# vincenthz/eccoxide

Hardware: AMD Instinct MI355X
Metric: variable-base scalarmuls/sec (batch) per GPU + achieved HBM GB/s vs roofline (higher is better)
Workload: dtype u32

## Files before the change

__graft_entry__.py:

```python
import os
import subprocess
import sys

ROOT = os.path.dirname(os.path.abspath(__file__))
if ROOT not in sys.path:
    sys.path.insert(0, ROOT)


def build() -> None:
    jobs = str(min(6, os.cpu_count() or 1))
    subprocess.check_call(["make", "-C", os.path.join(ROOT, "eccoxide_amd", "csrc"), "-j", jobs, "ARCH=gfx950"])
    subprocess.check_call(["make", "-C", os.path.join(ROOT, "oracle")])
    subprocess.check_call(["make", "-C", os.path.join(ROOT, "tests", "cpp")])
    subprocess.check_call(["make", "-C", os.path.join(ROOT, "tests", "hip")])
    subprocess.check_call(["make", "-C", os.path.join(ROOT, "tests", "hip_p256k1")])
    subprocess.check_call(["make", "-C", os.path.join(ROOT, "tests", "hip_ed25519")])
    subprocess.check_call(["make", "-C", os.path.join(ROOT, "tests", "hip_merged")])
    subprocess.check_call(["make", "-C", os.path.join(ROOT, "tests", "hip_signed")])
    subprocess.check_call(["make", "-C", os.path.join(ROOT, "tests", "hip_lo32")])
    subprocess.check_call(["make", "-C", os.path.join(ROOT, "tests", "hip_ecdsa")])
    subprocess.check_call(["make", "-C", os.path.join(ROOT, "tests", "hip_ed25519_sign")])
    subprocess.check_call(["make", "-C", os.path.join(ROOT, "tests", "hip_ecdsa_sign")])
    subprocess.check_call(["make", "-C", os.path.join(ROOT, "tests", "hip_h2c")])
    subprocess.check_call(["make", "-C", os.path.join(ROOT, "tests", "hip_g2")])
    subprocess.check_call(["make", "-C", os.path.join(ROOT, "tests", "hip_h2c_g2")])
    import eccoxide_amd
    from eccoxide_amd import _lib

    lib = _lib.load()
    assert lib.eccx_field_bytes(eccoxide_amd.P256R1) == 32


def smoke() -> None:
    import eccoxide_amd as E
    from eccoxide_amd import workload as W
    from tests import oracle_lib

    ora = oracle_lib.load()
    with E.Engine(0) as eng:
        for curve, n in (("p256r1", 300), ("ed25519", 300)):
            ks = W.random_scalars(curve, n, seed=1).tobytes()
            want_b = ora.base(curve, ks, threads=4)
            got_b = eng.scalarmul_base(curve, ks)
            assert got_b[0] == want_b[0] and got_b[1] == want_b[1], f"{curve}: fixed-base mismatch vs oracle"
            pts = want_b[0]
            ks2 = W.random_scalars(curve, n, seed=2).tobytes()
            want_v = ora.var(curve, ks2, pts, threads=4)
            got_d = eng.scalarmul_var(curve, ks2, pts)
            assert got_d[0] == want_v[0] and got_d[1] == want_v[1], f"{curve}: variable-base mismatch vs oracle"
            got_v = eng.scalarmul_var(curve, ks2, pts, want_proj=True)
            assert got_v[0] == want_v[0] and got_v[1] == want_v[1], f"{curve}: mirror variable-base mismatch vs oracle"
            assert got_v[2] == want_v[2], f"{curve}: un-normalised coordinates differ from the reference algorithm"
            for kw in ({"ct_scan": True}, {"ct_gather": True}):
                got_c = eng.scalarmul_base(curve, ks, **kw)
                assert got_c[0] == want_b[0] and got_c[1] == want_b[1], f"{curve} {kw}: secret-scalar fixed base mismatch vs oracle"
            got_c = eng.scalarmul_var(curve, ks2, pts, ct_scan=True)
            assert got_c[0] == want_v[0] and got_c[1] == want_v[1], f"{curve}: secret-scalar variable base mismatch vs oracle"
            from oracle import ecc_ref as R

            inf = None if curve == "ed25519" else got_d[1]
            enc = eng.point_compress(curve, got_d[0], inf)
            assert enc == R.point_compress_bytes(curve, got_d[0], inf), f"{curve}: point encoding differs from the oracle"
            back = eng.point_decompress(curve, enc)
            assert back[0] == got_d[0] and back[1] == (bytes(n) if inf is None else inf), f"{curve}: decompress(compress(P)) != P"
        curve, n = "bls12_381_g1", 200
        pts = ora.base(curve, W.random_scalars(curve, n, seed=3).tobytes(), threads=4)[0]
        ks = W.random_scalars(curve, n, seed=4).tobytes()
        want = ora.var(curve, ks, pts, threads=4)
        for opts in ({}, {"assume_subgroup": True}, {"ct_scan": True}, {"ct_scan": True, "assume_subgroup": True}):
            got = eng.scalarmul_var(curve, ks, pts, **opts)
            assert got[0] == want[0] and got[1] == want[1], f"{curve} {opts}: variable-base mismatch vs oracle"
# ... 58 lines not shown
```

eccoxide_amd/csrc/kernels_coz.hpp:

```cpp
#pragma once
#include <type_traits>
#include "inv_gcd.hpp"
#include "kernels_ct.hpp"

namespace eccx {

struct NoGlv {
  static constexpr int K_BITS = 0;
};
struct PrimeOrderBases : NoGlv {};

template <class G>
ECCX_DEV void glv_split(uint32_t (&k1)[5], uint32_t (&k2)[5], const uint8_t* __restrict__ kb) {
  uint32_t k[8];
#pragma unroll
  for (int i = 0; i < 8; ++i) {
    const uint8_t* b = kb + 28 - 4 * i;
    k[i] = ((uint32_t)b[0] << 24) | ((uint32_t)b[1] << 16) | ((uint32_t)b[2] << 8) | (uint32_t)b[3];
  }
  uint32_t prod[13];
#pragma unroll
  for (int i = 0; i < 13; ++i) prod[i] = 0;
#pragma unroll
  for (int i = 0; i < 8; ++i) {
// ... 156 lines not shown
    }
  }
  s1 = h1[4] >> 31;
  s2 = h2[4] >> 31;
  uint32_t c_1 = s1, c_2 = s2;
#pragma unroll
  for (int i = 0; i < 5; ++i) {
    const uint64_t a = (uint64_t)(h1[i] ^ (0u - s1)) + c_1;
    k1[i] = (uint32_t)a;
    c_1 = (uint32_t)(a >> 32);
    const uint64_t b = (uint64_t)(h2[i] ^ (0u - s2)) + c_2;
    k2[i] = (uint32_t)b;
    c_2 = (uint32_t)(b >> 32);
  }
}


template <class CU>
constexpr int urowc_words() { return ((3 * CU::N + 3) / 4) * 4; }

template <class CU>
ECCX_DEV void u2_load(U<CU, 1, 3>& x, U<CU, 1, 3>& y, const uint32_t* __restrict__ row) {
  constexpr int N = CU::N;
  constexpr int W = ((2 * N + 3) / 4) * 4;
  uint32_t w[W];
  const uint4* src = reinterpret_cast<const uint4*>(row);
#pragma unroll
  for (int i = 0; i < W / 4; ++i) {
    const uint4 q = src[i];
    w[4 * i] = q.x; w[4 * i + 1] = q.y; w[4 * i + 2] = q.z; w[4 * i + 3] = q.w;
  }
#pragma unroll
  for (int i = 0; i < N; ++i) { x.v[i] = w[i]; y.v[i] = w[N + i]; }
}

template <class CU>
constexpr int urow2_words() { return ((2 * CU::N + 3) / 4) * 4; }
#ifndef ECCX_CT_VAR_PK
#define ECCX_CT_VAR_PK 0
#endif
template <class CU, bool TAGGED = false>
ECCX_DEV void u2_store(uint32_t* __restrict__ row, const U<CU, 1, 3>& x, const U<CU, 1, 3>& y) {
  constexpr int N = CU::N;
  constexpr int W = urow2_words<CU>();
  constexpr uint32_t T = TAGGED ? CT_F32_TAG : 0u;
  uint32_t w[W];
#pragma unroll
  for (int i = 0; i < W; ++i) w[i] = (i < N ? x.v[i] : (i < 2 * N ? y.v[i - N] : 0u)) | T;
  uint4* dst = reinterpret_cast<uint4*>(row);
#pragma unroll
  for (int i = 0; i < W / 4; ++i) dst[i] = make_uint4(w[4 * i], w[4 * i + 1], w[4 * i + 2], w[4 * i + 3]);
}

template <class CU>
ECCX_DEV void ujac_madd_signed(UJac<CU>& r, bool& h_zero, bool& r_zero, const UJac<CU>& p,
                          const U<CU, 1, 3>& x2, const U<CU, 1, 3>& y2, bool neg) {
  auto z1z1 = u_sqr(p.z);
  auto u2 = u_mul(x2, z1z1);
  auto t = u_mul(p.z, z1z1);
  U<CU, 2, 4> sy;
  u_select(sy, neg, u_neg(y2), u_as<2, 4>(y2));
  auto s2 = u_mul(u_reduce(sy), t);
  auto h = u_reduce(u_sub(u2, p.x));
  auto rr = u_reduce(u_sub(s2, p.y));
  h_zero = u_is_zero_mod_p(h);
  r_zero = u_is_zero_mod_p(rr);
  auto hh = u_sqr(h);
  auto hhh = u_mul(h, hh);
  auto v = u_mul(p.x, hh);
  auto r2 = u_sqr(rr);
  auto x3 = u_reduce(u_sub(u_sub(u_sub(r2, hhh), v), v));
  r.x = x3;
  if constexpr (CU::KIND == UK_MONT) {
    r.y = u_fit<1, 3>(u_mul_add(rr, u_sub(v, x3), u_neg(p.y), hhh));
  } else if constexpr (UB<CU>::SPARSE) {
    r.y = u_mul_sub(rr, u_sub(v, x3), p.y, hhh);
  } else if constexpr (UBS<CU>::DENSE) {
    r.y = u_mul_sub(rr, u_sdiff(v, x3), p.y, hhh);
  } else {
    auto y3a = u_mul(rr, u_sub(v, x3));
    auto y1h = u_mul(p.y, hhh);
    r.y = u_reduce(u_sub(y3a, y1h));
  }
  r.z = u_fit<UJac<CU>::ZK, UJac<CU>::ZV>(u_mul(p.z, h));
}

template <class CU>
ECCX_DEV void uzaddu(U<CU, 1, 3>& x1, U<CU, 1, 3>& y1, U<CU, 1, 3>& x2, U<CU, 1, 3>& y2, U<CU, 1, 3>& d_out, bool& d_zero) {
  const auto d = u_reduce(u_sub(x1, x2));
  d_zero = u_is_zero_mod_p(d);
  const auto c = u_sqr(d);
  const U<CU, 1, 3> w1 = u_fit<1, 3>(u_mul(x1, c));
  const auto w2 = u_mul(x2, c);
  const auto e = u_reduce(u_sub(y1, y2));
  const auto dd = u_sqr(e);
  const U<CU, 1, 3> a1 = u_fit<1, 3>(u_mul(y1, u_sub(w1, w2)));
  const auto x3 = u_reduce(u_sub(u_sub(dd, w1), w2));
  const auto y3m = u_mul(e, u_sub(w1, x3));
  x2 = x3;
  y2 = u_reduce(u_sub(y3m, a1));
  x1 = w1;
  y1 = a1;
  d_out = d;
}

template <class CU>
ECCX_DEV void ujac_madd_ct(UJac<CU>& r, bool& h_zero, bool& r_zero, const UJac<CU>& p, const U<CU, 1, 3>& x2,
                           const U<CU, 1, 3>& y2) {
  auto z1z1 = u_sqr(p.z);
  auto u2 = u_mul(x2, z1z1);
  auto t = u_mul(p.z, z1z1);
  auto s2 = u_mul(y2, t);
  auto h = u_reduce(u_sub(u2, p.x));
  auto rr = u_reduce(u_sub(s2, p.y));
  h_zero = u_is_zero_mod_p_ct(h);
  r_zero = u_is_zero_mod_p_ct(rr);
  auto hh = u_sqr(h);
  auto hhh = u_mul(h, hh);
  auto v = u_mul(p.x, hh);
  auto r2 = u_sqr(rr);
  auto x3 = u_reduce(u_sub(u_sub(u_sub(r2, hhh), v), v));
  r.x = x3;
  if constexpr (CU::KIND == UK_MONT) {
    r.y = u_fit<1, 3>(u_mul_add(rr, u_sub(v, x3), u_neg(p.y), hhh));
  } else if constexpr (UB<CU>::SPARSE) {
    r.y = u_mul_sub(rr, u_sub(v, x3), p.y, hhh);
  } else {
    auto y3a = u_mul(rr, u_sub(v, x3));
    auto y1h = u_mul(p.y, hhh);
    r.y = u_reduce(u_sub(y3a, y1h));
  }
  r.z = u_fit<UJac<CU>::ZK, UJac<CU>::ZV>(u_mul(p.z, h));
}

template <class CU>
ECCX_DEV void ujac_dbl_affine(U<CU, 1, 3>& x3, U<CU, 1, 3>& y3, U<CU, 1, 3>& z3, U<CU, 1, 3>& sv, U<CU, 1, 3>& y8v,
                              const U<CU, 1, 3>& px, const U<CU, 1, 3>& py) {
// ... 28 lines not shown
  constexpr int NWIN = (8 * CS::SB + 1 + WB - 1) / WB;
  return (CS::PRIME_ORDER || ASSUME_PRIME) ? (8 * CS::SB - CS::NBITS + 1) / WB + 1 : NWIN;
}
#ifndef ECCX_CT_VAR_BITS
#define ECCX_CT_VAR_BITS 4
#endif

#ifndef ECCX_COZ_OCC_U14
#define ECCX_COZ_OCC_U14 3
#endif
#ifndef ECCX_COZ_OCC_BLS
#define ECCX_COZ_OCC_BLS 2
#endif
#ifndef ECCX_COZ_OCC_U9
#define ECCX_COZ_OCC_U9 4
#endif
#ifndef ECCX_COZ_NESTED_LADDER
#define ECCX_COZ_NESTED_LADDER 1
#endif
template <class CU, bool GLV>
constexpr int coz_occupancy() {
  return CU::N <= 9 ? ECCX_COZ_OCC_U9
                    : (CU::N <= 14 ? (GLV ? ECCX_OCC_U14 : (CU::KIND == UK_MONT ? ECCX_COZ_OCC_BLS : ECCX_COZ_OCC_U14)) : ECCX_OCC_U18);
}


template <class CU, class G, bool GLV, bool FUSED = false, int WB = 5, bool CT = false>
__global__ void __launch_bounds__(WG, (coz_occupancy<CU, GLV>())) k_scalarmul_coz_unsat(size_t n, const uint8_t* __restrict__ scalars,
                                                                                 const uint8_t* __restrict__ points,
                                                                                 uint32_t* __restrict__ rows_out,
                                                                                 uint8_t* __restrict__ flags,
                                                                                 uint32_t* __restrict__ scratch, uint32_t opts,
                                                                                 const uint8_t* __restrict__ base_scalars = nullptr,
                                                                                 const uint32_t* __restrict__ utable = nullptr) {
  static_assert(!(GLV && FUSED), "the verify shape takes any curve point");
  static_assert(!(CT && FUSED), "the verify shape has no secret-scalar form");
  constexpr bool ASSUME_PRIME = std::is_same<G, PrimeOrderBases>::value;
  constexpr bool LATTICE = GlvLattice<G>::value;
  static_assert(!(LATTICE && CT), "the secret-scalar endomorphism ladder is written for the unsigned split");
  static_assert(!ASSUME_PRIME || CT, "PrimeOrderBases only narrows the secret-scalar form's collision windows");
  static_assert(WB >= 3 && WB <= 5, "table rows 1 .. 2^(WB-1) must fit the slab");
  constexpr int TBL = 1 << (WB - 1);
  using CS = typename CU::Sat;
  constexpr bool ISO = CS::A0 == 1;
  constexpr int L = CS::L;
  constexpr int N = CU::N;
  constexpr int FB = CS::FB;
  constexpr int SB = CS::SB;
  static_assert(!GLV || SB == 32, "the split is written for 256-bit scalars");
  constexpr int NWIN = GLV ? (G::K_BITS + 1 + WB - 1) / WB : (8 * SB + 1 + WB - 1) / WB;
  constexpr int S = (!GLV && !CT) ? (8 * SB + 1) % WB : 0;
  constexpr int NWIN_MAIN = S != 0 ? (8 * SB + 1) / WB : NWIN;
  constexpr bool SHARED_INV = !ISO && !CT;
  static_assert(WG == 256, "the shared inversion multiplies the values of four waves");
  constexpr int WR = urowc_words<CU>();
  static_assert(!ISO || WR >= 16 + N, "row 0 holds the split scalar and zeta");
  using T = U<CU, 1, 3>;
  uint32_t* slab = scratch + ((size_t)blockIdx.x * FAST_TABLE_ROWS * WG + threadIdx.x) * (size_t)WR;
  auto row = [&](uint32_t e) { return slab + (size_t)e * WG * WR; };
  constexpr int WC = urow2_words<CU>();
  static_assert(!CT || (size_t)TBL * WC <= (size_t)(FAST_TABLE_ROWS - 1 - TBL) * WR, "the compact table must fit the free rows");
  uint32_t* cslab = scratch + ((size_t)blockIdx.x * FAST_TABLE_ROWS + (TBL + 1)) * WG * (size_t)WR + (size_t)threadIdx.x * WC;
  auto crow = [&](uint32_t e) { return cslab + (size_t)(e - 1) * WG * WC; };
  uint32_t iter = 0u;
  for (size_t base = (size_t)blockIdx.x * WG; base < n; base += (size_t)gridDim.x * WG, ++iter) {
    const size_t gid = base + threadIdx.x;
    const bool active = gid < n;
    const size_t idx = active ? gid : n - 1;
    const uint8_t* __restrict__ k = scalars + idx * (size_t)SB;
    if constexpr (GLV) {
      uint32_t k1[5], k2[5], s1 = 0, s2 = 0;
      if constexpr (LATTICE) glv_split_lattice<G>(k1, k2, s1, s2, k);
      else glv_split<G>(k1, k2, k);
      uint4* d = reinterpret_cast<uint4*>(row(0));
      d[0] = make_uint4(k1[0], k1[1], k1[2], k1[3]);
      d[1] = make_uint4(k1[4], s1, 0u, 0u);
      d[2] = make_uint4(k2[0], k2[1], k2[2], k2[3]);
      d[3] = make_uint4(k2[4], s2, 0u, 0u);
    }
    const uint32_t* kw = row(0);

    T one;
#pragma unroll
    for (int i = 0; i < N; ++i) one.v[i] = CU::ONE[i];
    UJac<CU> q;
    bool rejected = false;
    {
      Fe<L> rx, ry;
      fe_load_be<CS>(rx, points + idx * (size_t)(2 * FB));
      fe_load_be<CS>(ry, points + idx * (size_t)(2 * FB) + FB);
      if (opts & OPT_VALIDATE) {
        Fe<L> mx, my;
        fe_to_mont<CS>(mx, rx);
        fe_to_mont<CS>(my, ry);
        rejected = !(fe_is_canonical<CS>(rx) && fe_is_canonical<CS>(ry) && on_curve<CS>(mx, my));
      }
      q.x = u_as<1, 3>(u_to_mont<CU>(rx));
      q.y = u_as<1, 3>(u_to_mont<CU>(ry));
    }
    if constexpr (FUSED) {
      if (opts & OPT_NEGATE_B) q.y = u_reduce(u_neg(q.y));
    }
    q.z = u_as<UJac<CU>::ZK, UJac<CU>::ZV>(one);
    u3_store<CU>(row(1), q.x, q.y, one);

    auto booth = [&](int w, bool second, uint32_t& d, bool& neg) {
// ... 49 lines not shown
          __shared__ uint32_t zsh[N][WG];
          const uint32_t tid = threadIdx.x;
          T zs;
          u_select(zs, degenerate, one, zacc);
#pragma unroll
          for (int i = 0; i < N; ++i) zsh[i][tid] = zs.v[i];
          __syncthreads();
          if ((uint32_t)__builtin_amdgcn_readfirstlane((int)(tid >> 6)) == (iter & 3u)) {
            const uint32_t col = tid & 63u;
            auto get = [&](int j) {
              T a;
#pragma unroll
              for (int i = 0; i < N; ++i) a.v[i] = zsh[i][col + 64u * j];
              return a;
            };
            auto put = [&](int j, const T& a) {
#pragma unroll
              for (int i = 0; i < N; ++i) zsh[i][col + 64u * j] = a.v[i];
            };
            const T p1 = u_fit<1, 3>(u_mul(get(0), get(1)));
            const T p2 = u_fit<1, 3>(u_mul(p1, get(2)));
            Fe<L> c;
            u_to_canonical<CU>(c, u_mul(p2, get(3)));
            fe_inv_gcd<CS>(c, c);
            T inv = u_as<1, 3>(u_to_mont<CU>(c));
            {
              const T a3 = get(3);
              put(3, u_fit<1, 3>(u_mul(inv, p2)));
              inv = u_fit<1, 3>(u_mul(inv, a3));
            }
            {
              const T a2 = get(2);
              put(2, u_fit<1, 3>(u_mul(inv, p1)));
              inv = u_fit<1, 3>(u_mul(inv, a2));
            }
            const T a0 = get(0), a1 = get(1);
            put(0, u_fit<1, 3>(u_mul(inv, a1)));
            put(1, u_fit<1, 3>(u_mul(inv, a0)));
          }
          __syncthreads();
#pragma unroll
          for (int i = 0; i < N; ++i) lam.v[i] = zsh[i][tid];
          __syncthreads();
        } else {
          Fe<L> c;
          u_to_canonical<CU>(c, zacc);
          fe_inv_gcd<CS>(c, c);
          lam = u_as<1, 3>(u_to_mont<CU>(c));
        }
        const T l2 = u_fit<1, 3>(u_sqr(lam));
        const T l3 = u_fit<1, 3>(u_mul(l2, lam));
        const T xt = u_fit<1, 3>(u_mul(tx, l2)), yt = u_fit<1, 3>(u_mul(ty, l3));
        if constexpr (CT) u2_store<CU, (ECCX_CT_VAR_PK != 0)>(crow(TBL), xt, yt);
        else u3_store<CU>(row(TBL), xt, yt, one);
      }
      for (int d = TBL - 1; d >= 1; --d) {
        lam = u_fit<1, 3>(u_mul(lam, next));
        T x, y;
        u3_load<CU>(x, y, next, row(d));
        const T l2 = u_fit<1, 3>(u_sqr(lam));
        const T l3 = u_fit<1, 3>(u_mul(l2, lam));
        const T xs = u_fit<1, 3>(u_mul(x, l2));
        const T ys = u_fit<1, 3>(u_mul(y, l3));
        if constexpr (CT) u2_store<CU, (ECCX_CT_VAR_PK != 0)>(crow(d), xs, ys);
        else if constexpr (GLV) u3_store<CU>(row(d), xs, ys, u_fit<1, 3>(u_mul_k<CU>(xs, CU::BETA)));
        else u3_store<CU>(row(d), xs, ys, one);
      }
      if constexpr (ISO) {
        uint32_t* zdst = row(0) + 16;
#pragma unroll
        for (int i = 0; i < N; ++i) zdst[i] = lam.v[i];
      }
    }

    if constexpr (CT) {
      constexpr int FULLW = GLV ? 1 : coz_full_windows<CU, WB, ASSUME_PRIME>();
      constexpr int HALVES = GLV ? 2 : 1;
      auto lookup = [&](int w, bool second, T& ex, T& ey, uint32_t& d) {
        bool neg;
        booth(w, second, d, neg);
        neg = neg != second;
#if ECCX_CT_VAR_PK
        {
          uint64_t acc[N];
#pragma unroll
          for (int p = 0; p < N; ++p) acc[p] = 0;
#pragma unroll 2
          for (int j = 1; j <= TBL; ++j) {
            uint32_t m;
            asm("v_cndmask_b32_e64 %0, 0, 1.0, %1" : "=v"(m) : "s"(__builtin_amdgcn_uicmp(d, (uint32_t)j, 32 )));
            const uint64_t m2 = m;
            const uint4* src = reinterpret_cast<const uint4*>(crow(j));
            uint4 v[WC / 4];
#pragma unroll
            for (int c = 0; c < WC / 4; ++c) v[c] = src[c];
#pragma unroll
            for (int p = 0; p < N; ++p) {
              const uint4 qv = v[p / 2];
              ct_fsel2(acc[p], (p & 1) ? (((uint64_t)qv.w << 32) | qv.z) : (((uint64_t)qv.y << 32) | qv.x), m2);
            }
          }
#pragma unroll
          for (int i = 0; i < N; ++i) {
            ex.v[i] = (uint32_t)(acc[i / 2] >> (32 * (i & 1))) & ~CT_F32_TAG;
            ey.v[i] = (uint32_t)(acc[(N + i) / 2] >> (32 * ((N + i) & 1))) & ~CT_F32_TAG;
          }
        }
#else
        u_set_zero(ex);
        u_set_zero(ey);
#pragma unroll 2
        for (int j = 1; j <= TBL; ++j) {
          T cx, cy;
          u2_load<CU>(cx, cy, crow(j));
          const uint64_t m = __builtin_amdgcn_uicmp(d, (uint32_t)j, 32 );
          u_cmov_ct(ex, m, cx);
          u_cmov_ct(ey, m, cy);
        }
// ... 13 lines not shown
        uint32_t d;
        lookup(NWIN - 1, false, ex, ey, d);
        q.x = ex;
        q.y = ey;
        u_select_ct(q.z, d == 0, u_as<UJac<CU>::ZK, UJac<CU>::ZV>(zero), u_as<UJac<CU>::ZK, UJac<CU>::ZV>(one));
      }
#pragma unroll 1
      for (int win = NWIN - 1; win >= 0; --win) {
        if (win != NWIN - 1) {
#pragma unroll 1
          for (int j = 0; j < WB; ++j) {
            UJac<CU> t;
            ujac_dbl<CU>(t, q);
            q = t;
          }
        }
#pragma unroll 1
        for (int half = (win == NWIN - 1) ? 1 : 0; half < HALVES; ++half) {
          T ex, ey;
          uint32_t d;
          lookup(win, half != 0, ex, ey, d);
          const bool q_inf = u_limbs_all_zero(q.z);
          const bool e_skip = d == 0;
          UJac<CU> sum;
          bool hz, rz;
          ujac_madd_ct<CU>(sum, hz, rz, q, ex, ey);
          if (win < FULLW) {
            T dx, dy, dz, sv, y8v;
            ujac_dbl_affine<CU>(dx, dy, dz, sv, y8v, ex, ey);
            const bool same_x = hz & !q_inf & !e_skip;
            const uint64_t mt = ct_mask(same_x & rz);
            const uint64_t mc = ct_mask(same_x & !rz);
            u_cmov_ct(sum.x, mt, dx);
            u_cmov_ct(sum.y, mt, dy);
            u_cmov_ct(sum.z, mt, TZ(u_as<UJac<CU>::ZK, UJac<CU>::ZV>(dz)));
            u_cmov_ct(sum.z, mc, TZ(u_as<UJac<CU>::ZK, UJac<CU>::ZV>(zero)));
          }
          const uint64_t mi = ct_mask(q_inf), mk = ct_mask(!e_skip);
          u_cmov_ct(sum.x, mi, ex);
          u_cmov_ct(sum.y, mi, ey);
          u_cmov_ct(sum.z, mi, TZ(u_as<UJac<CU>::ZK, UJac<CU>::ZV>(one)));
          u_cmov_ct(q.x, mk, sum.x);
          u_cmov_ct(q.y, mk, sum.y);
          u_cmov_ct(q.z, mk, sum.z);
        }
      }
    } else {
      constexpr int WIN_END = S != 0 ? -1 : 0;
      {
        uint32_t d;
        bool neg;
        booth(NWIN_MAIN - 1, false, d, neg);
        T tx, ty;
        u2_load<CU>(tx, ty, row(d ? d : 1));
        U<CU, 2, 4> sy;
        u_select(sy, neg, u_neg(ty), u_as<2, 4>(ty));
        q.x = tx;
        q.y = u_reduce(sy);
        q.z = u_as<UJac<CU>::ZK, UJac<CU>::ZV>(one);
        if (d == 0) u_set_zero(q.z);
      }
      bool fix_lane = false;
      auto dbl_step = [&](bool fix) __attribute__((always_inline)) {
        UJac<CU> t;
        if constexpr (UBS<CU>::DENSE) {
          ujac_dbl_merged<CU>(t, q);
          if (fix) {
            const uint64_t keep = ct_mask(!fix_lane);
            u_cmov_ct(t.x, keep, q.x);
            u_cmov_ct(t.y, keep, q.y);
            u_cmov_ct(t.z, keep, q.z);
          }
          q = t;
        } else {
          ujac_dbl<CU>(t, q);
          if (fix) {
            u_select(q.x, fix_lane, t.x, q.x);
            u_select(q.y, fix_lane, t.y, q.y);
            u_select(q.z, fix_lane, t.z, q.z);
          } else {
            q = t;
          }
        }
      };
      auto add_step = [&](int win, bool second) __attribute__((always_inline)) -> bool {
        uint32_t d;
        bool neg;
        booth(win, second, d, neg);
        if (second && !LATTICE) neg = !neg;
        T ex, ey;
        if constexpr (GLV) {
          T eb;
          u3_load<CU>(ex, ey, eb, row(d ? d : 1));
          if (second) ex = eb;
        } else {
          u2_load<CU>(ex, ey, row(d ? d : 1));
        }
        const bool q_inf = u_limbs_all_zero(q.z);
        const bool e_skip = (d == 0);
        UJac<CU> sum;
        bool hz, rz;
        ujac_madd_signed<CU>(sum, hz, rz, q, ex, ey, neg);
        const bool same_x = hz && !q_inf && !e_skip;
        fix_lane = same_x && rz;
        if (same_x && !rz) u_set_zero(sum.z);
        if (__builtin_amdgcn_ballot_w64(q_inf) != 0) {
          U<CU, 2, 4> sy;
          u_select(sy, neg, u_neg(ey), u_as<2, 4>(ey));
          u_select(sum.x, q_inf, ex, sum.x);
          u_select(sum.y, q_inf, u_reduce(sy), sum.y);
          u_select(sum.z, q_inf, u_as<UJac<CU>::ZK, UJac<CU>::ZV>(one), sum.z);
        }
        const bool keep = e_skip || fix_lane;
        u_select(q.x, keep, q.x, sum.x);
        u_select(q.y, keep, q.y, sum.y);
        u_select(q.z, keep, q.z, sum.z);
        return __builtin_amdgcn_ballot_w64(fix_lane) != 0;
      };
      if constexpr (!GLV && ECCX_COZ_NESTED_LADDER) {
#pragma unroll 1
        for (int win = NWIN_MAIN - 2; win >= WIN_END; --win) {
          const int nd = (S != 0 && win < 0) ? S : WB;
#pragma unroll 1
          for (int sub = 0; sub < nd; ++sub) dbl_step(false);
          if (add_step(win, false)) dbl_step(true);
        }
      } else {
        int win, sub;
        if constexpr (GLV) {
          win = NWIN_MAIN - 1;
          sub = WB + 1;
        } else {
          win = NWIN_MAIN - 2;
          sub = 0;
        }
        bool fix_pending = false;
        while (win >= WIN_END) {
          const int nd = (S != 0 && win < 0) ? S : WB;
          bool step_done;
          if (fix_pending || sub < nd) {
            dbl_step(fix_pending);
            fix_pending = false;
            step_done = true;
          } else {
            fix_pending = add_step(win, GLV && sub == WB + 1);
            step_done = !fix_pending;
          }
          if (step_done) {
            if (sub < nd + (GLV ? 1 : 0)) {
              ++sub;
            } else {
              sub = 0;
              --win;
            }
          }
        }
      }
    }
    if constexpr (ISO) {
      T zeta;
      const uint32_t* zsrc = row(0) + 16;
#pragma unroll
      for (int i = 0; i < N; ++i) zeta.v[i] = zsrc[i];
// ... 12 lines not shown
```

eccoxide_amd/csrc/ufe.hpp:

```cpp
#pragma once
#include "fe.hpp"

#include <type_traits>

#ifndef ECCX_SOLINAS_REDUCE
#define ECCX_SOLINAS_REDUCE 1
#endif

namespace eccx {

#include "umad_chunks.inc"

__device__ __forceinline__ void smad1_k(uint64_t& acc, uint32_t a, int32_t k) {
  asm("v_mad_i64_i32 %0, vcc, %1, %2, %0" : "+v"(acc) : "v"(a), "s"(k) : "vcc");
}

__device__ __forceinline__ void smad1_v(uint64_t& acc, int32_t a, int32_t b) {
  asm("v_mad_i64_i32 %0, vcc, %1, %2, %0" : "+v"(acc) : "v"(a), "v"(b) : "vcc");
}

template <int S>
__device__ __forceinline__ void ucarry_hi(uint64_t& acc) {
  uint64_t r;
  asm("v_mad_u64_u32 %0, vcc, %1, %2, 0" : "=&v"(r) : "v"((uint32_t)(acc >> 32)), "n"(1 << S) : "vcc");
// ... 421 lines not shown
  for (int i = 0; i < N; ++i) r[i] = t[i];
}

template <class C, bool NEG_SQ, class TB = uint32_t>
ECCX_DEV void u_mul_sub_core_pp1(uint32_t (&r)[C::N], const uint32_t (&a)[C::N], const TB (&b)[C::N],
                                 const uint32_t (&c)[C::N], const uint32_t (&d)[C::N]) {
  constexpr int N = C::N;
  constexpr bool BS = std::is_same_v<TB, int32_t>;
  static_assert(BS || std::is_same_v<TB, uint32_t>, "second factor: unsigned limbs or signed differences");
  static_assert(C::KIND == UK_MONT_PP1 && C::SPARSE_N == 0, "p = -1 mod 2^B with p + 1 as plain digits");
  uint32_t m[N], t[N];
  int32_t nc[N];
#pragma unroll
  for (int i = 0; i < N; ++i) nc[i] = NEG_SQ ? -(int32_t)(c[i] << 1) : -(int32_t)c[i];
  uint64_t acc = 0;
  std::conditional_t<BS, UMacQS<32 - C::B>, UMacQC<false, 32 - C::B>> qa;
  UMacQ<true> qm;
#pragma unroll
  for (int k = 0; k < 2 * N - 1; ++k) {
    const int lo = k < N ? 0 : k - N + 1, hi = k < N ? k : N - 1;
    if (k >= N && C::P[k - N] != 0) acc += (uint64_t)C::P[k - N];
#pragma unroll
    for (int i = lo; i <= hi; ++i) qa.push(acc, a[i], b[k - i]);
    qa.flush(acc);
    if constexpr (NEG_SQ) {
#pragma unroll
      for (int i = lo; 2 * i < k; ++i) smad1_v(acc, nc[i], (int32_t)(c[k - i] << 1));
      if ((k & 1) == 0) smad1_v(acc, nc[k / 2], (int32_t)c[k / 2]);
    } else {
#pragma unroll
      for (int i = lo; i <= hi; ++i) smad1_v(acc, nc[i], (int32_t)d[k - i]);
    }
#pragma unroll
    for (int i = lo; i <= (k < N ? k - 1 : N - 1); ++i) {
      if (C::PP1[k - i] != 0) qm.push(acc, m[i], C::PP1[k - i]);
    }
    qm.flush(acc);
    if (k < N - 1) {
      m[k] = (uint32_t)acc;
      if constexpr (BS) qa.carry(acc);
      else qa.carry(acc, true);
      continue;
    }
    if (k < N) m[k] = (uint32_t)acc & C::MASK;
    else t[k - N] = (uint32_t)acc & C::MASK;
    acc = (uint64_t)((int64_t)acc >> C::B);
  }
  acc += (uint64_t)C::P[N - 1];
  t[N - 1] = (uint32_t)acc;
#pragma unroll
  for (int i = 0; i < N; ++i) r[i] = t[i];
}

template <class C, bool SQR, bool BCONST>
ECCX_DEV void u_mul_core_mers(uint32_t (&r)[C::N], const uint32_t (&a)[C::N], const uint32_t (&b)[C::N]) {
  constexpr int N = C::N;
  constexpr int S = C::B * N - C::PBITS;
  static_assert(S >= 1 && S <= 2, "wrap factor must keep shifted limbs below 2^32");
  uint32_t t[N], bw[N], a2[N];
#pragma unroll
  for (int i = 0; i < N; ++i) {
    if constexpr (SQR) {
      a2[i] = a[i] << 1;
      bw[i] = (S == 1) ? 0u : a[i] << (S + 1);
    } else {
      a2[i] = 0;
      bw[i] = b[i] << S;
    }
  }
  uint64_t acc = 0;
  UMacQ<BCONST && !SQR> qa;
  UMacQ<false> qw;
#pragma unroll
  for (int k = 0; k < N; ++k) {
    if constexpr (SQR) {
#pragma unroll
      for (int i = 0; 2 * i < k; ++i) qa.push(acc, a[i], a2[k - i]);
      if ((k & 1) == 0) qa.push(acc, a[k / 2], a[k / 2]);
      qa.flush(acc);
#pragma unroll
      for (int i = k + 1; 2 * i < k + N; ++i) {
        if constexpr (S == 1) qw.push(acc, a2[i], a2[k + N - i]);
        else qw.push(acc, a[i], bw[k + N - i]);
      }
      if (((k + N) & 1) == 0) {
        if constexpr (S == 1) qw.push(acc, a[(k + N) / 2], a2[(k + N) / 2]);
        else qw.push(acc, a2[(k + N) / 2], a2[(k + N) / 2]);
      }
      qw.flush(acc);
    } else {
#pragma unroll
      for (int i = 0; i <= k; ++i) qa.push(acc, a[i], b[k - i]);
      qa.flush(acc);
#pragma unroll
      for (int i = k + 1; i < N; ++i) qw.push(acc, a[i], bw[k + N - i]);
      qw.flush(acc);
    }
    t[k] = (uint32_t)acc & C::MASK;
    acc >>= C::B;
  }
  acc = (acc << S) + t[0];
  t[0] = (uint32_t)acc & C::MASK;
  t[1] += (uint32_t)(acc >> C::B);
#pragma unroll
  for (int i = 0; i < N; ++i) r[i] = t[i];
}
// ... 188 lines not shown
  static_assert(K1 * K2 <= UBS<C>::KKS && 2 * K3 * K3 <= UBS<C>::KKS, "a product overflows the signed columns");
  static_assert(UBS<C>::ks_ok(2 * K3), "doubled / negated operands must stay below 2^31");
  static_assert((uint32_t)(V1 * V2) < C::RP && (uint32_t)(2 * V3 * V3) < C::RP, "result outside (0, 3p)");
  U<C, 1, 3> r;
  if constexpr (UB<C>::SPARSE) u_mul_sub_core_sparse<C, true>(r.v, a.v, b.v, c.v, c.v);
  else if constexpr (UBS<C>::DENSE) u_mul_sub_core_pp1<C, true>(r.v, a.v, b.v, c.v, c.v);
  else u_mul_sub_core_mont<C, true>(r.v, a.v, b.v, c.v, c.v);
  return r;
}

template <class C, int K, int V>
struct US {
  static_assert(K >= 1 && UBS<C>::ks_ok(K), "signed limbs must stay below 2^31");
  static_assert(V >= 1 && V <= 4096, "value bound out of range");
  int32_t v[C::N];
};

template <class C, int V1, int V2>
ECCX_DEV auto u_sdiff(const U<C, 1, V1>& a, const U<C, 1, V2>& b) {
  US<C, 1, (V1 > V2 ? V1 : V2)> r;
#pragma unroll
  for (int i = 0; i < C::N; ++i) r.v[i] = (int32_t)(a.v[i] - b.v[i]);
  return r;
}

template <class C>
constexpr bool ubs_neg_side_ok(int kk) {
  return (uint64_t)C::N * (uint64_t)kk * UB<C>::COL <= (~(uint64_t)0 >> 1) - ((uint64_t)1 << (64 - C::B));
}

template <class C, int K1, int V1, int K2, int V2, int K3, int V3, int K4, int V4>
ECCX_DEV auto u_mul_sub(const U<C, K1, V1>& a, const US<C, K2, V2>& b, const U<C, K3, V3>& c, const U<C, K4, V4>& d) {
  static_assert(UBS<C>::DENSE, "signed operands are implemented for p = -1 mod 2^B with p + 1 as plain digits");
  static_assert(K1 * K2 <= UBS<C>::KKS && K3 * K4 <= UBS<C>::KKS, "a product overflows the signed columns");
  static_assert(UBS<C>::ks_ok(K1) && UBS<C>::ks_ok(K3) && UBS<C>::ks_ok(K4), "negated / signed operands must stay below 2^31");
  static_assert(ubs_neg_side_ok<C>(K1 * K2 + K3 * K4), "the negative side of a column overflows");
  static_assert((uint32_t)(V1 * V2 + V3 * V4) < C::RP, "result outside (0, 3p)");
  U<C, 1, 3> r;
  u_mul_sub_core_pp1<C, false, int32_t>(r.v, a.v, b.v, c.v, d.v);
  return r;
}
template <class C, int K1, int V1, int K2, int V2, int K3, int V3>
ECCX_DEV auto u_mul_sub_2sqr(const U<C, K1, V1>& a, const US<C, K2, V2>& b, const U<C, K3, V3>& c) {
  static_assert(UBS<C>::DENSE, "signed operands are implemented for p = -1 mod 2^B with p + 1 as plain digits");
  static_assert(K1 * K2 <= UBS<C>::KKS && 2 * K3 * K3 <= UBS<C>::KKS, "a product overflows the signed columns");
  static_assert(UBS<C>::ks_ok(K1) && UBS<C>::ks_ok(2 * K3), "doubled / negated operands must stay below 2^31");
  static_assert(ubs_neg_side_ok<C>(K1 * K2 + 2 * K3 * K3), "the negative side of a column overflows");
  static_assert((uint32_t)(V1 * V2 + 2 * V3 * V3) < C::RP, "result outside (0, 3p)");
  U<C, 1, 3> r;
  u_mul_sub_core_pp1<C, true, int32_t>(r.v, a.v, b.v, c.v, c.v);
  return r;
}

template <class C, int V1>
ECCX_DEV auto u_sqr2(const U<C, 1, V1>& a) {
  static_assert(UBS<C>::DENSE && UB<C>::LO32, "written for p = -1 mod 2^B with p + 1 as plain digits");
  static_assert(UB<C>::kk_ok(2, 1), "columns: a square with doubled terms carries a product with K1*K2 = 2");
  static_assert(UB<C>::KMAX >= 2, "limbs: the doubled operand a << 1 (below 2 * 2^B) stays below 2^32");
  static_assert(UB<C>::vout(2 * V1, V1) <= 3, "result too large: reduce the operand first");
  U<C, 1, UB<C>::vout(2 * V1, V1)> r;
  u_mul_core_mont<C, true, false, true, true>(r.v, a.v, a.v);
  return r;
}

template <class C, int K1, int V1>
ECCX_DEV auto u_sqr(const U<C, K1, V1>& a) {
  if constexpr (!UB<C>::ksq_ok(K1) || (UB<C>::vout(V1, V1) > 3)) {
    return u_sqr(u_reduce(a));
  } else {
    U<C, 1, UB<C>::vout(V1, V1)> r;
    u_mul_core<C, true, false>(r.v, a.v, a.v);
    return r;
  }
}

template <class C, int K1, int V1>
ECCX_DEV auto u_mul_k(const U<C, K1, V1>& a, const uint32_t (&k)[C::N]) {
  if constexpr (!UB<C>::kk_ok(K1, 1) || (UB<C>::vout(V1, 1) > 3)) {
    return u_mul_k(u_reduce(a), k);
  } else {
    U<C, 1, UB<C>::vout(V1, 1)> r;
    u_mul_core<C, false, true>(r.v, a.v, k);
    return r;
  }
}

template <class C>
ECCX_DEV U<C, 1, 2> u_mul_k_exit(const U<C, 1, 3>& a, const uint32_t (&k)[C::N]) {
  static_assert(UB<C>::MONT && UB<C>::vout(3, 1) <= 2, "Montgomery fields; a reduced operand times a constant below p");
  U<C, 1, 2> r;
  u_mul_core_mont<C, false, true, false>(r.v, a.v, k);
  return r;
}

template <class C, int K1, int V1>
ECCX_DEV U<C, 1, 2> u_mul_small(const U<C, K1, V1>& a, uint32_t k) {
  static_assert(C::KIND == UK_PM19, "written for 2^255 - 19");
  constexpr int N = C::N;
  uint32_t t[N];
  uint64_t acc = 0;
#pragma unroll
  for (int i = 0; i < N; ++i) {
    umad1_v(acc, a.v[i], k);
    t[i] = (uint32_t)acc & C::MASK;
    acc >>= C::B;
  }
// ... 208 lines not shown
```

Measured before the change: 78.34 million.

## Store negated y in table rows and use signed differences in mixed add

Precomputed table rows for the variable-base path now hold -y in the third slot, so the Booth-signed lookup just picks the y pointer instead of negating and reducing per window. The mixed Jacobian addition uses unsigned-free signed differences (h, r) fed directly into new signed-multiply/square cores, skipping reductions. Zero tests on h and r take a cheap limb-0 filter first and fall back to a full reduce only when some lane in the wave might be zero. This cuts per-addition field reductions and negations, at the cost of new signed arithmetic kernels, extra table-build work, and possible extra register pressure.

```diff
diff --git a/__graft_entry__.py b/__graft_entry__.py
--- a/__graft_entry__.py
+++ b/__graft_entry__.py
@@ -17,6 +17,7 @@
     subprocess.check_call(["make", "-C", os.path.join(ROOT, "tests", "hip_ed25519")])
     subprocess.check_call(["make", "-C", os.path.join(ROOT, "tests", "hip_merged")])
     subprocess.check_call(["make", "-C", os.path.join(ROOT, "tests", "hip_signed")])
+    subprocess.check_call(["make", "-C", os.path.join(ROOT, "tests", "hip_signed_hr")])
     subprocess.check_call(["make", "-C", os.path.join(ROOT, "tests", "hip_lo32")])
     subprocess.check_call(["make", "-C", os.path.join(ROOT, "tests", "hip_ecdsa")])
     subprocess.check_call(["make", "-C", os.path.join(ROOT, "tests", "hip_ed25519_sign")])
diff --git a/eccoxide_amd/csrc/kernels_coz.hpp b/eccoxide_amd/csrc/kernels_coz.hpp
--- a/eccoxide_amd/csrc/kernels_coz.hpp
+++ b/eccoxide_amd/csrc/kernels_coz.hpp
@@ -232,15 +232,35 @@
   for (int i = 0; i < W / 4; ++i) dst[i] = make_uint4(w[4 * i], w[4 * i + 1], w[4 * i + 2], w[4 * i + 3]);
 }
 
+#ifndef ECCX_COZ_SIGNED_ROWS
+#define ECCX_COZ_SIGNED_ROWS 1
+#endif
+#ifndef ECCX_COZ_SIGNED_HR
+#define ECCX_COZ_SIGNED_HR 1
+#endif
+
 template <class CU>
-ECCX_DEV void ujac_madd_signed(UJac<CU>& r, bool& h_zero, bool& r_zero, const UJac<CU>& p,
-                          const U<CU, 1, 3>& x2, const U<CU, 1, 3>& y2, bool neg) {
+ECCX_DEV void ujac_madd_entry(UJac<CU>& r, bool& h_zero, bool& r_zero, const UJac<CU>& p,
+                              const U<CU, 1, 3>& x2, const U<CU, 1, 3>& y2) {
   auto z1z1 = u_sqr(p.z);
   auto u2 = u_mul(x2, z1z1);
   auto t = u_mul(p.z, z1z1);
-  U<CU, 2, 4> sy;
-  u_select(sy, neg, u_neg(y2), u_as<2, 4>(y2));
-  auto s2 = u_mul(u_reduce(sy), t);
+  auto s2 = u_mul(y2, t);
+  if constexpr (UBS<CU>::DENSE && ECCX_COZ_SIGNED_HR) {
+    const auto h = u_sdiff(u2, p.x);
+    const auto rr = u_sdiff(s2, p.y);
+    h_zero = u_sdiff_is_zero_mod_p(h, u2, p.x);
+    r_zero = u_sdiff_is_zero_mod_p(rr, s2, p.y);
+    auto hh = u_sqr(h);
+    auto hhh = u_mul(hh, h);
+    auto v = u_mul(p.x, hh);
+    auto r2 = u_sqr(rr);
+    auto x3 = u_reduce(u_sub(u_sub(u_sub(r2, hhh), v), v));
+    r.x = x3;
+    r.y = u_mul_sub(rr, u_sdiff(v, x3), p.y, hhh);
+    r.z = u_fit<UJac<CU>::ZK, UJac<CU>::ZV>(u_mul(p.z, u_sub(u2, p.x)));
+    return;
+  }
   auto h = u_reduce(u_sub(u2, p.x));
   auto rr = u_reduce(u_sub(s2, p.y));
   h_zero = u_is_zero_mod_p(h);
@@ -263,6 +283,22 @@
     r.y = u_reduce(u_sub(y3a, y1h));
   }
   r.z = u_fit<UJac<CU>::ZK, UJac<CU>::ZV>(u_mul(p.z, h));
+}
+
+template <class CU>
+ECCX_DEV void ujac_madd_signed(UJac<CU>& r, bool& h_zero, bool& r_zero, const UJac<CU>& p,
+                          const U<CU, 1, 3>& x2, const U<CU, 1, 3>& y2, bool neg) {
+  U<CU, 2, 4> sy;
+  u_select(sy, neg, u_neg(y2), u_as<2, 4>(y2));
+  ujac_madd_entry<CU>(r, h_zero, r_zero, p, x2, u_reduce(sy));
+}
+
+template <class CU>
+ECCX_DEV void u2_load_signed(U<CU, 1, 3>& x, U<CU, 1, 3>& y, const uint32_t* __restrict__ row, bool neg) {
+  constexpr int N = CU::N;
+  const uint32_t* __restrict__ ys = row + (neg ? 2 * N : N);
+#pragma unroll
+  for (int i = 0; i < N; ++i) { x.v[i] = row[i]; y.v[i] = ys[i]; }
 }
 
 template <class CU>
@@ -397,6 +433,7 @@
   constexpr int S = (!GLV && !CT) ? (8 * SB + 1) % WB : 0;
   constexpr int NWIN_MAIN = S != 0 ? (8 * SB + 1) / WB : NWIN;
   constexpr bool SHARED_INV = !ISO && !CT;
+  constexpr bool SROWS = ECCX_COZ_SIGNED_ROWS && UBS<CU>::DENSE && !GLV && !CT && !ISO;
   static_assert(WG == 256, "the shared inversion multiplies the values of four waves");
   constexpr int WR = urowc_words<CU>();
   static_assert(!ISO || WR >= 16 + N, "row 0 holds the split scalar and zeta");
@@ -552,6 +589,7 @@
         const T l3 = u_fit<1, 3>(u_mul(l2, lam));
         const T xt = u_fit<1, 3>(u_mul(tx, l2)), yt = u_fit<1, 3>(u_mul(ty, l3));
         if constexpr (CT) u2_store<CU, (ECCX_CT_VAR_PK != 0)>(crow(TBL), xt, yt);
+        else if constexpr (SROWS) u3_store<CU>(row(TBL), xt, yt, u_reduce(u_neg(yt)));
         else u3_store<CU>(row(TBL), xt, yt, one);
       }
       for (int d = TBL - 1; d >= 1; --d) {
@@ -564,6 +602,7 @@
         const T ys = u_fit<1, 3>(u_mul(y, l3));
         if constexpr (CT) u2_store<CU, (ECCX_CT_VAR_PK != 0)>(crow(d), xs, ys);
         else if constexpr (GLV) u3_store<CU>(row(d), xs, ys, u_fit<1, 3>(u_mul_k<CU>(xs, CU::BETA)));
+        else if constexpr (SROWS) u3_store<CU>(row(d), xs, ys, u_reduce(u_neg(ys)));
         else u3_store<CU>(row(d), xs, ys, one);
       }
       if constexpr (ISO) {
@@ -683,11 +722,16 @@
         bool neg;
         booth(NWIN_MAIN - 1, false, d, neg);
         T tx, ty;
-        u2_load<CU>(tx, ty, row(d ? d : 1));
-        U<CU, 2, 4> sy;
-        u_select(sy, neg, u_neg(ty), u_as<2, 4>(ty));
+        if constexpr (SROWS) {
+          u2_load_signed<CU>(tx, ty, row(d ? d : 1), neg);
+        } else {
+          u2_load<CU>(tx, ty, row(d ? d : 1));
+          U<CU, 2, 4> sy;
+          u_select(sy, neg, u_neg(ty), u_as<2, 4>(ty));
+          ty = u_reduce(sy);
+        }
         q.x = tx;
-        q.y = u_reduce(sy);
+        q.y = ty;
         q.z = u_as<UJac<CU>::ZK, UJac<CU>::ZV>(one);
         if (d == 0) u_set_zero(q.z);
       }
@@ -724,6 +768,8 @@
           T eb;
           u3_load<CU>(ex, ey, eb, row(d ? d : 1));
           if (second) ex = eb;
+        } else if constexpr (SROWS) {
+          u2_load_signed<CU>(ex, ey, row(d ? d : 1), neg);
         } else {
           u2_load<CU>(ex, ey, row(d ? d : 1));
         }
@@ -731,15 +777,21 @@
         const bool e_skip = (d == 0);
         UJac<CU> sum;
         bool hz, rz;
-        ujac_madd_signed<CU>(sum, hz, rz, q, ex, ey, neg);
+        if constexpr (SROWS) ujac_madd_entry<CU>(sum, hz, rz, q, ex, ey);
+        else ujac_madd_signed<CU>(sum, hz, rz, q, ex, ey, neg);
         const bool same_x = hz && !q_inf && !e_skip;
         fix_lane = same_x && rz;
         if (same_x && !rz) u_set_zero(sum.z);
         if (__builtin_amdgcn_ballot_w64(q_inf) != 0) {
-          U<CU, 2, 4> sy;
-          u_select(sy, neg, u_neg(ey), u_as<2, 4>(ey));
-          u_select(sum.x, q_inf, ex, sum.x);
-          u_select(sum.y, q_inf, u_reduce(sy), sum.y);
+          if constexpr (SROWS) {
+            u_select(sum.x, q_inf, ex, sum.x);
+            u_select(sum.y, q_inf, ey, sum.y);
+          } else {
+            U<CU, 2, 4> sy;
+            u_select(sy, neg, u_neg(ey), u_as<2, 4>(ey));
+            u_select(sum.x, q_inf, ex, sum.x);
+            u_select(sum.y, q_inf, u_reduce(sy), sum.y);
+          }
           u_select(sum.z, q_inf, u_as<UJac<CU>::ZK, UJac<CU>::ZV>(one), sum.z);
         }
         const bool keep = e_skip || fix_lane;
diff --git a/eccoxide_amd/csrc/ufe.hpp b/eccoxide_amd/csrc/ufe.hpp
--- a/eccoxide_amd/csrc/ufe.hpp
+++ b/eccoxide_amd/csrc/ufe.hpp
@@ -497,6 +497,52 @@
   for (int i = 0; i < N; ++i) r[i] = t[i];
 }
 
+template <class C, bool SQR>
+ECCX_DEV void u_smul_core_pp1(uint32_t (&r)[C::N], const uint32_t (&a)[C::N], const int32_t (&b)[C::N]) {
+  constexpr int N = C::N;
+  static_assert(C::KIND == UK_MONT_PP1 && C::SPARSE_N == 0, "p = -1 mod 2^B with p + 1 as plain digits");
+  uint32_t m[N], t[N];
+  int32_t b2[N];
+  if constexpr (SQR) {
+#pragma unroll
+    for (int i = 0; i < N; ++i) b2[i] = (int32_t)((uint32_t)b[i] << 1);
+  }
+  uint64_t acc = 0;
+  UMacQS<32 - C::B> qa;
+  UMacQ<true> qm;
+#pragma unroll
+  for (int k = 0; k < 2 * N - 1; ++k) {
+    const int lo = k < N ? 0 : k - N + 1, hi = k < N ? k : N - 1;
+    if constexpr (!SQR) {
+      if (k >= N && C::P[k - N] != 0) acc += (uint64_t)C::P[k - N];
+#pragma unroll
+      for (int i = lo; i <= hi; ++i) qa.push(acc, a[i], b[k - i]);
+    } else {
+#pragma unroll
+      for (int i = lo; 2 * i < k; ++i) qa.push(acc, (uint32_t)b[i], b2[k - i]);
+      if ((k & 1) == 0) qa.push(acc, (uint32_t)b[k / 2], b[k / 2]);
+    }
+    qa.flush(acc);
+#pragma unroll
+    for (int i = lo; i <= (k < N ? k - 1 : N - 1); ++i) {
+      if (C::PP1[k - i] != 0) qm.push(acc, m[i], C::PP1[k - i]);
+    }
+    qm.flush(acc);
+    if (k < N - 1) {
+      m[k] = (uint32_t)acc;
+      qa.carry(acc);
+      continue;
+    }
+    if (k < N) m[k] = (uint32_t)acc & C::MASK;
+    else t[k - N] = (uint32_t)acc & C::MASK;
+    acc = (uint64_t)((int64_t)acc >> C::B);
+  }
+  if constexpr (!SQR) acc += (uint64_t)C::P[N - 1];
+  t[N - 1] = (uint32_t)acc;
+#pragma unroll
+  for (int i = 0; i < N; ++i) r[i] = t[i];
+}
+
 template <class C, bool SQR, bool BCONST>
 ECCX_DEV void u_mul_core_mers(uint32_t (&r)[C::N], const uint32_t (&a)[C::N], const uint32_t (&b)[C::N]) {
   constexpr int N = C::N;
@@ -791,6 +837,61 @@
   return r;
 }
 
+template <class C, int K1, int V1, int K2, int V2, int K3, int V3, int K4, int V4>
+ECCX_DEV auto u_mul_sub(const US<C, K1, V1>& a, const US<C, K2, V2>& b, const U<C, K3, V3>& c, const U<C, K4, V4>& d) {
+  static_assert(UBS<C>::DENSE, "signed operands are implemented for p = -1 mod 2^B with p + 1 as plain digits");
+  static_assert(K1 * K2 <= UBS<C>::KKS && K3 * K4 <= UBS<C>::KKS, "a product overflows the signed columns");
+  static_assert(UBS<C>::ks_ok(K3) && UBS<C>::ks_ok(K4), "negated / signed operands must stay below 2^31");
+  static_assert(ubs_neg_side_ok<C>(K1 * K2 + K3 * K4), "the negative side of a column overflows");
+  static_assert((uint32_t)(V1 * V2 + V3 * V4) < C::RP, "result outside (0, 3p)");
+  uint32_t au[C::N];
+#pragma unroll
+  for (int i = 0; i < C::N; ++i) au[i] = (uint32_t)a.v[i];
+  U<C, 1, 3> r;
+  u_mul_sub_core_pp1<C, false, int32_t>(r.v, au, b.v, c.v, d.v);
+  return r;
+}
+
+template <class C, int K1, int V1, int K2, int V2>
+ECCX_DEV auto u_mul(const U<C, K1, V1>& a, const US<C, K2, V2>& b) {
+  static_assert(UBS<C>::DENSE && UB<C>::LO32, "signed operands are implemented for p = -1 mod 2^B with p + 1 as plain digits");
+  static_assert(K1 * K2 <= UBS<C>::KKS, "the product overflows the signed columns");
+  static_assert(UBS<C>::ks_ok(K1), "the unsigned factor's limbs enter as signed: they must stay below 2^31");
+  static_assert(ubs_neg_side_ok<C>(K1 * K2), "the negative side of a column overflows");
+  static_assert((uint32_t)(V1 * V2) < C::RP, "result outside (0, 3p)");
+  U<C, 1, 3> r;
+  u_smul_core_pp1<C, false>(r.v, a.v, b.v);
+  return r;
+}
+
+template <class C, int K, int V>
+ECCX_DEV auto u_sqr(const US<C, K, V>& a) {
+  static_assert(UBS<C>::DENSE && UB<C>::LO32, "signed operands are implemented for p = -1 mod 2^B with p + 1 as plain digits");
+  static_assert(K * K <= UBS<C>::KKS, "the square overflows the signed columns");
+  static_assert(UBS<C>::ks_ok(2 * K), "doubled signed limbs must stay below 2^31");
+  static_assert(ubs_neg_side_ok<C>(K * K), "the negative side of a column overflows");
+  static_assert(UB<C>::vout(V, V) <= 3, "result too large");
+  U<C, 1, UB<C>::vout(V, V)> r;
+  uint32_t unused[C::N] = {};
+  u_smul_core_pp1<C, true>(r.v, unused, a.v);
+  return r;
+}
+
+template <class C, int V1, int V2, int V>
+ECCX_DEV bool u_sdiff_is_zero_mod_p(const US<C, 1, V>& d, const U<C, 1, V1>& a, const U<C, 1, V2>& b) {
+  static_assert(C::KIND == UK_MONT_PP1 && V1 <= 3 && V2 <= 3, "p = -1 mod 2^B; operands below 3p");
+  static_assert(C::N == 9, "the pin below is written out for nine limbs");
+  const bool pass = (((uint32_t)d.v[0] + 2u) & C::MASK) <= 4u;
+  bool zero = false;
+  if (__builtin_amdgcn_ballot_w64(pass) != 0) {
+    U<C, 1, V1> ao = a;
+    asm volatile("" : "+v"(ao.v[0]), "+v"(ao.v[1]), "+v"(ao.v[2]), "+v"(ao.v[3]), "+v"(ao.v[4]), "+v"(ao.v[5]), "+v"(ao.v[6]),
+                      "+v"(ao.v[7]), "+v"(ao.v[8]));
+    zero = pass && u_is_zero_mod_p_ct(u_reduce(u_sub(ao, b)));
+  }
+  return zero;
+}
+
 template <class C, int V1>
 ECCX_DEV auto u_sqr2(const U<C, 1, V1>& a) {
   static_assert(UBS<C>::DENSE && UB<C>::LO32, "written for p = -1 mod 2^B with p + 1 as plain digits");
```

Measured after the change: 79.45 million (median of 6 runs). +1.4%, better.
